# jgkellymit/GENIE-SMEM

Hardware: NVIDIA B200
Metric: SMEM reads/sec (BWA-SMEM; LUT/RMI under methods) (higher is better)
Workload: dtype u32

## Files before the change

genie_smem_b200/_capi.py:

```python
import ctypes as C
import os

_HERE = os.path.dirname(os.path.abspath(__file__))
LIB_PATH = os.path.join(_HERE, "libgenie_smem.so")

OK, E_INVALID, E_NOMEM, E_CUDA, E_CAPACITY, E_NODEVICE = 0, -1, -2, -3, -4, -5
METHOD_BWA, METHOD_LUT, METHOD_RMI = 0, 1, 2
READ_OK, READ_REF_RAISES, READ_TOO_SHORT = 0, 1, 2

u8p, u32p, u64p, i64p, f64p = (C.POINTER(t) for t in (C.c_uint8, C.c_uint32, C.c_uint64, C.c_int64, C.c_double))


class IndexInfo(C.Structure):
    _fields_ = [("n_bases", C.c_uint64), ("n_rows", C.c_uint64), ("n_buckets", C.c_uint64), ("bucket_bytes", C.c_uint64),
                ("text_words", C.c_uint64), ("count", C.c_uint32 * 4), ("C", C.c_uint32 * 5), ("primary_fwd", C.c_uint32),
                ("primary_rev", C.c_uint32), ("has_reverse", C.c_uint32), ("reserved", C.c_uint32)]


class DevIndex(C.Structure):
    _fields_ = [("n_rows", C.c_uint64), ("n_buckets", C.c_uint64), ("fwd_buckets", C.c_void_p), ("rev_buckets", C.c_void_p),
                ("sa", C.c_void_p), ("text2bit", C.c_void_p), ("C", C.c_uint32 * 5), ("primary_fwd", C.c_uint32),
                ("primary_rev", C.c_uint32), ("seed_K", C.c_uint32), ("seed_table", C.c_void_p)]


# ... 47 lines not shown
    "gsm_pack_reads": (C.c_int, [C.c_char_p, C.c_void_p, C.c_uint64, C.c_void_p, C.c_void_p]),
    "gsm_text_pack_device": (C.c_int, [C.c_void_p, C.c_uint64, C.c_uint32, C.c_void_p, C.c_void_p, C.c_void_p]),
    "gsm_index_build_device_workspace": (C.c_int, [C.c_uint64, C.c_uint32, C.POINTER(C.c_uint64)]),
    "gsm_index_build_device": (C.c_int, [C.c_void_p, C.c_uint64, C.c_uint32, C.c_void_p, C.c_void_p, C.c_void_p, C.c_void_p, C.c_uint64,
                                         C.POINTER(IndexInfo), C.c_void_p]),
    "gsm_fastq_scan": (C.c_int, [C.c_void_p, C.c_uint64, C.POINTER(C.c_uint64), C.c_void_p, C.c_void_p, C.c_uint64, C.c_uint32]),
    "gsm_fastq_gather": (C.c_int, [C.c_void_p, C.c_void_p, C.c_void_p, C.c_uint64, C.c_void_p, C.c_void_p, C.c_uint32]),
    "gsm_pack_reads_device": (C.c_int, [C.c_void_p, C.c_void_p, C.c_uint32, C.c_void_p, C.c_uint64, C.c_uint32, C.c_void_p, C.c_void_p, C.c_void_p,
                                        C.c_void_p]),
    "gsm_fastq_count_device": (C.c_int, [C.c_void_p, C.c_uint64, C.c_void_p, C.c_void_p]),
    "gsm_fastq_records_device": (C.c_int, [C.c_void_p, C.c_uint64, C.c_void_p, C.c_uint64, C.c_void_p, C.c_void_p, C.c_void_p, C.c_void_p]),
    "gsm_pack_reads_scattered_device": (C.c_int, [C.c_void_p, C.c_void_p, C.c_void_p, C.c_void_p, C.c_uint64, C.c_uint32, C.c_void_p, C.c_void_p,
                                                  C.c_void_p]),
    "gsm_pack_reads_device_check": (C.c_int, [C.c_void_p, C.c_void_p]),
    "gsm_reads_both_strands_device": (C.c_int, [C.POINTER(DevReads), C.c_void_p, C.c_void_p, C.c_void_p, C.c_void_p]),
    "gsm_smem_workspace_info": (C.c_int, [C.c_uint64, C.c_uint32, C.POINTER(WorkspaceInfo)]),
    "gsm_backsearch_batch": (C.c_int, [C.POINTER(DevIndex), C.POINTER(DevReads), C.c_void_p, C.c_void_p, C.c_void_p]),
    "gsm_backsearch_add_one_batch": (C.c_int, [C.POINTER(DevIndex), C.c_uint64, C.c_void_p, C.c_void_p, C.c_void_p, C.c_void_p]),
    "gsm_sa_lookup_batch": (C.c_int, [C.POINTER(DevIndex), C.c_uint64, C.c_void_p, C.c_void_p, C.c_void_p]),
    "gsm_sa_sample_build": (C.c_int, [C.POINTER(DevIndex), C.c_uint32, C.c_void_p, C.c_void_p]),
    "gsm_locate_sampled_batch": (C.c_int, [C.POINTER(DevIndex), C.c_void_p, C.c_uint32, C.c_uint64, C.c_void_p, C.c_void_p, C.c_void_p]),
    "gsm_lut_build": (C.c_int, [C.POINTER(DevIndex), C.c_uint32, C.c_void_p, C.c_void_p]),
    "gsm_seed_table_build": (C.c_int, [C.POINTER(DevIndex), C.c_uint32, C.c_void_p, C.c_void_p]),
    "gsm_smem_batch": (C.c_int, [C.c_int, C.POINTER(DevIndex), C.POINTER(DevReads), C.c_uint32, C.c_uint32, C.c_void_p,
                                 C.POINTER(DevRmi), C.POINTER(Workspace), C.c_void_p]),
    "gsm_smem_sweep": (C.c_int, [C.POINTER(DevIndex), C.POINTER(DevReads), C.POINTER(Workspace), C.c_void_p]),
    "gsm_smem_select": (C.c_int, [C.c_int, C.POINTER(DevIndex), C.POINTER(DevReads), C.c_uint32, C.c_uint32, C.c_void_p,
                                  C.POINTER(DevRmi), C.POINTER(Workspace), C.c_void_p]),
    "gsm_smem_collect": (C.c_int, [C.POINTER(DevReads), C.POINTER(Workspace), C.c_void_p, C.c_uint64, C.c_void_p]),
    "gsm_rmi_probe_build": (C.c_int, [C.POINTER(DevIndex), C.c_void_p, C.c_void_p]),
    "gsm_rmi_bounds_build": (C.c_int, [C.POINTER(DevIndex), C.c_uint32, C.c_void_p, C.c_void_p]),
    "gsm_option_lut_frame_machine": (C.c_int, [C.c_int]),
    "gsm_option_rmi_prefilter": (C.c_int, [C.c_int]),
    "gsm_rmi_hazard_scan": (C.c_int, [C.POINTER(DevIndex), C.POINTER(DevRmi), C.c_void_p, C.c_uint64, C.c_void_p, C.POINTER(C.c_uint64), C.c_void_p]),
    "gsm_rmi_hazard_hash": (C.c_int, [C.c_void_p, C.c_uint64, C.c_void_p, C.c_uint32]),
    "gsm_rmi_none_rows": (C.c_int, [C.POINTER(DevIndex), C.c_uint32, C.c_void_p, C.c_void_p, C.c_void_p]),
    "gsm_rmi_lookup_batch": (C.c_int, [C.POINTER(DevIndex), C.POINTER(DevRmi), C.c_uint64, C.c_void_p, C.c_void_p, C.c_void_p,
                                       C.c_void_p, C.c_void_p, C.c_void_p]),
    "gsm_comm_unique_id": (C.c_int, [C.c_void_p]),
    "gsm_comm_init": (C.c_int, [C.c_void_p, C.c_int, C.c_int, C.POINTER(C.c_void_p)]),
    "gsm_comm_free": (C.c_int, [C.c_void_p]),
    "gsm_comm_info": (C.c_int, [C.c_void_p, C.POINTER(C.c_int), C.POINTER(C.c_int), C.POINTER(C.c_int)]),
    "gsm_comm_allgather_u64": (C.c_int, [C.c_void_p, C.c_void_p, C.c_uint64, C.c_void_p, C.c_void_p]),
    "gsm_gather_records": (C.c_int, [C.c_void_p, C.c_void_p, C.c_uint64, C.c_void_p, C.c_void_p, C.c_int, C.c_void_p]),
    "gsm_peer_export": (C.c_int, [C.c_void_p, C.c_void_p, C.POINTER(C.c_uint64)]),
    "gsm_peer_open": (C.c_int, [C.c_void_p, C.c_uint64, C.POINTER(C.c_void_p)]),
    "gsm_peer_close": (C.c_int, [C.c_void_p, C.c_uint64]),
    "gsm_smem_collect_gathered": (C.c_int, [C.POINTER(DevReads), C.POINTER(Workspace), C.c_void_p, C.c_uint64, C.c_void_p, C.c_uint32,
                                            C.c_void_p, C.c_void_p]),
# ... 47 lines not shown
```

genie_smem_b200/csrc/kernels.cu:

```cuda
#include <cuda_runtime.h>

#include <algorithm>
#include <cstdint>
#include <cstdio>
#include <cstdlib>
#include <cstring>
#include <string>
#include <type_traits>

#include "../../include/genie_smem.h"
#include "host_common.hpp"
#include "select_logic.cuh"
#include "sweep_device.cuh"


namespace gsm {

#define GSM_CUDA(call)                                                                          \
    do {                                                                                        \
        cudaError_t e__ = (call);                                                               \
        if (e__ != cudaSuccess)                                                                 \
            return fail(GSM_E_CUDA, std::string(#call) + ": " + cudaGetErrorString(e__));       \
    } while (0)

// ... 847 lines not shown
    }
    table[code] = make_uint2(lo, cnt);
}

__global__ void k_seed_build(const uint4* fwd, const uint4* rev, IndexMeta meta, uint32_t K, uint64_t n_codes, uint4* table) {
    const uint64_t code = (uint64_t)blockIdx.x * blockDim.x + threadIdx.x;
    if (code >= n_codes) return;
    auto lf = [fwd](uint64_t idx) { return ldg_half(fwd, idx); };
    auto lr = [rev](uint64_t idx) { return ldg_half(rev, idx); };
    uint32_t lo = 0, cnt = meta.n_rows, rlo = 0, rcnt = meta.n_rows;
    for (uint32_t t = 0; t < K; ++t) {
        const uint32_t c = (uint32_t)(code >> (2 * t)) & 3u;
        const StepOut r = step_single(lf, lo, lo + cnt, c, meta.C[c], meta.prim_f);
        lo = r.lo_new; cnt = r.cnt_new;
    }
    for (uint32_t t = 0; t < K && rcnt && cnt; ++t) {
        const uint32_t c = (uint32_t)(code >> (2 * (K - 1 - t))) & 3u;
        const StepOut r = step_single(lr, rlo, rlo + rcnt, c, meta.C[c], meta.prim_r);
        rlo = r.lo_new; rcnt = r.cnt_new;
    }
    table[code] = make_uint4(lo, cnt, cnt ? rlo : 0u, 0u);
}

__global__ void k_bounds_build(const uint4* fwd, IndexMeta meta, uint32_t K, uint64_t n_codes, const uint4* seed_tab, uint32_t seed_K,
                               uint2* table) {
    const uint64_t code = (uint64_t)blockIdx.x * blockDim.x + threadIdx.x;
    if (code >= n_codes) return;
    auto load = [fwd](uint64_t idx) { return ldg_half(fwd, idx); };
    uint32_t lo = 0, cnt = meta.n_rows, t = 0;
    if (seed_tab) {
        const uint4 e = __ldg(seed_tab + (code & ((1ull << (2u * seed_K)) - 1ull)));
        lo = e.x; cnt = e.y; t = seed_K;
    }
    for (; t < K; ++t) {
        const uint32_t c = (uint32_t)(code >> (2 * t)) & 3u;
        const StepOut r = step_single(load, lo, lo + cnt, c, meta.C[c], meta.prim_f);
        lo = r.lo_new; cnt = r.cnt_new;
    }
    table[code] = make_uint2(lo, cnt);
}

__global__ void k_rmi_lookup(const uint32_t* sa, const uint32_t* text, uint64_t n_rows, uint64_t n_bases, RmiModel m, uint64_t n,
                             const uint64_t* codes, double* pred, int64_t* lo, int64_t* hi, uint8_t* status) {
    const uint64_t i = (uint64_t)blockIdx.x * blockDim.x + threadIdx.x;
    if (i >= n) return;
    auto sal = [sa](uint64_t r) { return __ldg(sa + r); };
// ... 327 lines not shown
        v.accessPolicyWindow.base_ptr = const_cast<void*>(ptr);
        v.accessPolicyWindow.num_bytes = (size_t)(bytes < (uint64_t)max_win ? bytes : (uint64_t)max_win);
        v.accessPolicyWindow.hitRatio = bytes <= carve ? 1.0f : (float)carve / (float)bytes;
        v.accessPolicyWindow.hitProp = cudaAccessPropertyPersisting;
        v.accessPolicyWindow.missProp = cudaAccessPropertyStreaming;
    }
    GSM_CUDA(cudaStreamSetAttribute((cudaStream_t)stream, cudaStreamAttributeAccessPolicyWindow, &v));
    if (!(ptr && bytes)) GSM_CUDA(cudaCtxResetPersistingL2Cache());
    return GSM_OK;
}

int gsm_seed_table_build(const gsm_dev_index* ix, uint32_t K, void* table, void* stream) {
    if (!ix || !table || !ix->fwd_buckets || !ix->rev_buckets) return fail(GSM_E_INVALID, "gsm_seed_table_build: needs both bucket arrays");
    if (K < 1 || K > 14) return fail(GSM_E_INVALID, "gsm_seed_table_build: K must be in 1..14");
    int st = device_ready();
    if (st) return st;
    const uint64_t n_codes = 1ull << (2 * K);
    k_seed_build<<<(unsigned)((n_codes + 127) / 128), 128, 0, (cudaStream_t)stream>>>((const uint4*)ix->fwd_buckets, (const uint4*)ix->rev_buckets,
                                                                                    make_meta(ix), K, n_codes, (uint4*)table);
    GSM_CUDA(cudaGetLastError());
    return GSM_OK;
}

static int fill_rmi(const gsm_dev_rmi* rmi, RmiModel* m, uint64_t n_rows) {
    memset(m, 0, sizeof(*m));
    if (!rmi || !rmi->level_sizes || !rmi->coef || !rmi->intercept) return fail(GSM_E_INVALID, "RMI parameters missing");
    if (rmi->n_levels < 1 || rmi->n_levels > 8 || rmi->K < 1 || rmi->K > 32) return fail(GSM_E_INVALID, "RMI: 1..8 levels, K in 1..32");
    m->K = rmi->K; m->n_levels = rmi->n_levels; m->coef = rmi->coef; m->intercept = rmi->intercept;
    m->stride = rmi->param_stride ? rmi->param_stride : 1u;
    uint32_t off = 0;
    for (uint32_t l = 0; l < rmi->n_levels; ++l) { m->level_size[l] = rmi->level_sizes[l]; m->level_off[l] = off; off += rmi->level_sizes[l]; }
    if (rmi->none_rows && rmi->n_none_rows) {
        if (rmi->n_none_rows != rmi->K) return fail(GSM_E_INVALID, "RMI: none_rows must hold exactly K rows (gsm_rmi_none_rows)");
        rmi_set_none_rows(*m, rmi->none_rows, rmi->n_none_rows, n_rows);
    }
    return GSM_OK;
}

int gsm_rmi_none_rows(const gsm_dev_index* ix, uint32_t K, uint32_t* rows_host, uint32_t* scratch, void* stream) {
    if (!ix || !ix->sa || !rows_host || !scratch || K < 1 || K > 32) return fail(GSM_E_INVALID, "gsm_rmi_none_rows: needs sa on the device, K in 1..32");
    int st = device_ready();
    if (st) return st;
    if (ix->n_rows <= K) return fail(GSM_E_INVALID, "gsm_rmi_none_rows: reference shorter than K");
    cudaStream_t s_ = (cudaStream_t)stream;
    GSM_CUDA(cudaMemsetAsync(scratch, 0, 33 * sizeof(uint32_t), s_));
    k_none_rows<<<(unsigned)((ix->n_rows + 255) / 256), 256, 0, s_>>>(ix->sa, ix->n_rows, K, scratch);
// ... 74 lines not shown
    GSM_CUDA(cudaGetLastError());
    return GSM_OK;
}

static int smem_check(const gsm_dev_index* ix, const gsm_dev_reads* rd, gsm_workspace* ws, int* sb, int* lb) {
    if (!ix || !rd || !ws) return fail(GSM_E_INVALID, "null");
    if (!ix->fwd_buckets || !ix->rev_buckets) return fail(GSM_E_INVALID, "the SMEM kernels need both BWT directions on the device");
    if (rd->max_len == 0 || rd->max_len > 65535) return fail(GSM_E_INVALID, "max_len must be in 1..65535");
    if (rd->n_reads >= (1ull << 32)) return fail(GSM_E_INVALID, "at most 2^32-1 reads per batch");
    if (ws->mem_cap >= (1ull << 32) || ws->rec_cap >= (1ull << 32)) return fail(GSM_E_INVALID, "pool capacities must be < 2^32 entries");
    int st = device_ready();
    if (st) return st;
    if ((st = sweep_grid(rd->max_len, sb))) return st;
    if ((st = select_grid(lb))) return st;
    const uint64_t need_sweep = sweep_scratch_bytes(*sb, rd->max_len);
    const uint64_t need_sel = (uint64_t)*lb * SELECT_THREADS * (uint64_t)select_stage_stride(rd->max_len) * 16ull;
    if (ws->quad_scratch_bytes < need_sweep || ws->quad_scratch_bytes < need_sel) return fail(GSM_E_CAPACITY, "quad_scratch too small (see gsm_smem_workspace_info)");
    const uint64_t n_tiles = (rd->n_reads + SCAN_TILE - 1) / SCAN_TILE;
    if (ws->scan_tmp_bytes < (n_tiles + 2) * 8) return fail(GSM_E_CAPACITY, "scan_tmp too small");
    return GSM_OK;
}

int gsm_smem_sweep(const gsm_dev_index* ix, const gsm_dev_reads* rd, gsm_workspace* ws, void* stream_) {
    int sb = 0, lb = 0;
    int st = smem_check(ix, rd, ws, &sb, &lb);
    if (st) return st;
    cudaStream_t stream = (cudaStream_t)stream_;
    GSM_CUDA(cudaMemsetAsync(ws->counters, 0, 8 * sizeof(uint64_t), stream));
    if (rd->n_reads == 0) return GSM_OK;
    SweepArgs sa;
    sa.fwd = (const uint4*)ix->fwd_buckets; sa.rev = (const uint4*)ix->rev_buckets; sa.meta = make_meta(ix);
    sa.reads = (const uint4*)rd->packed; sa.chunk_off = rd->chunk_off; sa.len = rd->len; sa.n_reads = (uint32_t)rd->n_reads;
    sa.read_u4 = sweep_read_u4(rd->max_len); sa.pack_u4 = sweep_pack_u4(rd->max_len); sa.max_len = rd->max_len;
    sa.seed_tab = (const uint4*)ix->seed_table; sa.seed_K = ix->seed_table ? ix->seed_K : 0u;
    if (sa.seed_tab && (sa.seed_K < 1 || sa.seed_K > 16)) return fail(GSM_E_INVALID, "seed table K must be in 1..16");
    sa.mem_pool = (uint4*)ws->mem_pool; sa.mem_cap = ws->mem_cap; sa.mem_off = ws->mem_off; sa.mem_cnt = ws->mem_cnt;
    sa.scratch = (uint4*)ws->quad_scratch; sa.counters = (unsigned long long*)ws->counters;
    static const int uniq_env = getenv("GSM_SWEEP_UNIQ") ? atoi(getenv("GSM_SWEEP_UNIQ")) : 1;
    sa.sa = ix->sa; sa.text = ix->text2bit; sa.n_bases = (uint32_t)(ix->n_rows - 1);
    const bool uniq = uniq_env != 0 && ix->sa && ix->text2bit;
    const int kind = sweep_kind(rd->max_len);
    if (kind == SWEEP_LANE) {
        static const int stats = getenv("GSM_SWEEP_STATS") ? atoi(getenv("GSM_SWEEP_STATS")) : 0;
        static const int paired = getenv("GSM_SWEEP_PAIRED") ? atoi(getenv("GSM_SWEEP_PAIRED")) : 0;
        if (uniq && paired) { k_sweep1<false, true, SWEEP1_MIN_BLOCKS, false, true><<<sb, SWEEP1_THREADS, sweep1_smem_bytes(rd->max_len, false), stream>>>(sa); GSM_CUDA(cudaGetLastError()); return GSM_OK; }
        if (uniq && stats) k_sweep1<false, true, SWEEP1_MIN_BLOCKS, true><<<sb, SWEEP1_THREADS, sweep1_smem_bytes(rd->max_len, false), stream>>>(sa);
        else if (uniq && sweep_blocks_env() == 6) k_sweep1<false, true, 6><<<sb, SWEEP1_THREADS, sweep1_smem_bytes(rd->max_len, false), stream>>>(sa);
        else if (uniq && sweep_blocks_env() == 8) k_sweep1<false, true, 8><<<sb, SWEEP1_THREADS, sweep1_smem_bytes(rd->max_len, false), stream>>>(sa);
        else if (uniq) k_sweep1<false, true><<<sb, SWEEP1_THREADS, sweep1_smem_bytes(rd->max_len, false), stream>>>(sa);
        else k_sweep1<false, false><<<sb, SWEEP1_THREADS, sweep1_smem_bytes(rd->max_len, false), stream>>>(sa);
    } else if (kind == SWEEP_LANE_LONG) {
        if (uniq) k_sweep1<true, true><<<sb, SWEEP1_THREADS, sweep1_smem_bytes(rd->max_len, true), stream>>>(sa);
        else k_sweep1<true, false><<<sb, SWEEP1_THREADS, sweep1_smem_bytes(rd->max_len, true), stream>>>(sa);
    } else {
        k_sweep<<<sb, SWEEP_THREADS, sweep_smem_bytes(rd->max_len), stream>>>(sa);
    }
    GSM_CUDA(cudaGetLastError());
    return GSM_OK;
// ... 203 lines not shown
```

genie_smem_b200/csrc/sweep_device.cuh:

```cuda
#pragma once
#include <cuda_runtime.h>

#include "sweep_logic.cuh"

namespace gsm {

constexpr int SWEEP_THREADS = 128;
constexpr int SWEEP_LPR = 2;
constexpr int SWEEP_GROUPS = SWEEP_THREADS / SWEEP_LPR;
constexpr int SWEEP_CAP = 12;
constexpr int SWEEP_MIN_BLOCKS = 8;

constexpr uint32_t MEMS_ORDERED = 0x80000000u;
constexpr uint32_t MEMS_PICKED = 0x40000000u;
constexpr uint32_t MEMS_COUNT = 0x3FFFFFFFu;

struct SweepArgs {
    const uint4* fwd;
    const uint4* rev;
    IndexMeta meta;
    const uint4* reads;
    const uint32_t* chunk_off;
    const uint32_t* len;
    uint32_t n_reads;
    uint32_t read_u4;
    uint32_t pack_u4;
    uint32_t max_len;
    const uint4* seed_tab;
    uint32_t seed_K;
    uint4* mem_pool;
    unsigned long long mem_cap;
    uint32_t* mem_off;
    uint32_t* mem_cnt;
    uint4* scratch;
    unsigned long long* counters;
    const uint32_t* sa;
    const uint32_t* text;
    uint32_t n_bases;
};

extern __shared__ uint4 g_sweep_smem[];

__device__ __forceinline__ Half ldg_half(const uint4* halves_base, size_t half_index) {
    Half h;
    asm volatile("ld.global.nc.v8.u32 {%0,%1,%2,%3,%4,%5,%6,%7}, [%8];"
                 : "=r"(h.c0), "=r"(h.c1), "=r"(h.l0), "=r"(h.l1), "=r"(h.l2), "=r"(h.h0), "=r"(h.h1), "=r"(h.h2)
                 : "l"(halves_base + half_index * 2));
    return h;
}

__device__ __forceinline__ StepOut pair_step(const uint4* __restrict__ bk, uint32_t P0, uint32_t P1, uint32_t ch, uint32_t Cc,
// ... 99 lines not shown
        if (g == 0) { a.mem_off[rid] = (uint32_t)off; a.mem_cnt[rid] = n; }
    }
};

__host__ __device__ inline uint32_t sweep_read_u4(uint32_t max_len) { return (max_len + 15u) / 16u; }

__global__ void __launch_bounds__(SWEEP_THREADS, SWEEP_MIN_BLOCKS) k_sweep(const SweepArgs a) {
    const uint32_t lane = threadIdx.x & 31u;
    const uint32_t g = lane & 1u;
    const uint32_t pair_in_block = threadIdx.x >> 1;
    const uint32_t pair_u4 = SWEEP_CAP + a.read_u4 + a.pack_u4;
    const uint32_t p0 = pair_in_block * pair_u4;
    const size_t gp = (size_t)blockIdx.x * SWEEP_GROUPS + pair_in_block;
    DevSweepCtx ctx{a, p0, (p0 + SWEEP_CAP) * 16u, (p0 + SWEEP_CAP + a.read_u4) * 4u, a.scratch + gp * 2 * a.max_len,
                    a.scratch + gp * 2 * a.max_len + a.max_len, g, 3u << (lane & ~1u), lane & ~1u};
    Sweeper<DevSweepCtx> sw;
    for (;;) {
        const bool need = sw.next(ctx, a.meta);
        if (!__any_sync(0xFFFFFFFFu, need)) break;
        const bool is_seed = need && sw.pending_seed();
        const bool is_step = need && !is_seed;
        uint4 se = make_uint4(0u, 0u, 0u, 0u);
        if (is_seed) se = ldg_seed(a.seed_tab + sw.P0);
        const bool rev = sw.on_reverse();
        const StepOut r = pair_step(rev ? a.rev : a.fwd, sw.P0, sw.P0 + sw.cnt, sw.ch, a.meta.C[sw.ch & 3u],
                                    rev ? a.meta.prim_r : a.meta.prim_f, g, is_step);
        if (is_step) sw.consume(ctx, a.meta, r);
        else if (is_seed) sw.consume_seed(ctx, a.meta, SeedEntry{se.x, se.y, se.z, se.w});
    }
}

constexpr int SWEEP1_THREADS = 128;
constexpr int SWEEP1_CAP = 8;
constexpr int SWEEP1_MIN_BLOCKS = 7;

struct LanePartial {
    uint32_t eq0, lt0;
    bool have;
};

template <bool PAIRED>
__device__ __forceinline__ bool lane_step(const uint4* __restrict__ fwd, const uint4* __restrict__ rev, bool use_rev, uint32_t P0, uint32_t P1,
                                          uint32_t ch, uint32_t Cc, uint32_t primary, bool active, LanePartial& part, StepOut& out) {
    constexpr uint32_t FULLM = 0xFFFFFFFFu;
    uint32_t b0, r0, b1, r1;
    split192(P0, b0, r0);
// ... 223 lines not shown

template <bool LONG, bool UNIQ, int MB = SWEEP1_MIN_BLOCKS, bool STATS = false, bool PAIRED = false>
__global__ void __launch_bounds__(SWEEP1_THREADS, MB) k_sweep1(const SweepArgs a) {
    using Ctx = DevSweepCtx1<LONG, UNIQ>;
    const uint32_t lane_u4 = sweep1_lane_u4(a.max_len, LONG);
    const uint32_t p0 = threadIdx.x * lane_u4;
    const size_t gl = (size_t)blockIdx.x * SWEEP1_THREADS + threadIdx.x;
    Ctx ctx{a, p0, (p0 + SWEEP1_CAP) * 4u, a.scratch + gl * 2 * a.max_len, a.scratch + gl * 2 * a.max_len + a.max_len, nullptr, 0u, Ctx::NO_FIN};
    Sweeper<Ctx> sw;
    LanePartial part{0u, 0u, false};
    uint32_t n_it = 0, n_step = 0, n_seed = 0, n_text = 0;
    for (;;) {
        ctx.flush_finished();
        const bool need = sw.next(ctx, a.meta);
        if (__any_sync(0xFFFFFFFFu, ctx.fin_n != Ctx::NO_FIN)) ctx.flush_finished();
        if (!__any_sync(0xFFFFFFFFu, need)) break;
        const bool is_seed = need && sw.pending_seed();
        const bool is_word = UNIQ && need && sw.pending_word();
        const bool is_cmp = UNIQ && need && sw.pending_cmp();
        const bool is_step = need && !is_seed && !is_word && !is_cmp;
        if (STATS) { n_it++; n_step += is_step; n_seed += is_seed; n_text += is_word || is_cmp; }
        uint4 se = make_uint4(0u, 0u, 0u, 0u);
        if (is_seed) se = ldg_seed(a.seed_tab + sw.P0);
        uint32_t wv = 0u, matched = 0u;
        if (UNIQ && is_word) wv = __ldg(a.sa + sw.aux);
        if (UNIQ && is_cmp) {
            matched = ctx.match_forward(sw.cmp_text(), sw.cmp_read());
            const uint32_t mx = sw.cmp_max(a.n_bases);
            matched = matched < mx ? matched : mx;
        }
        const bool rev = sw.on_reverse();
        StepOut r;
        const bool stepped = lane_step<PAIRED>(a.fwd, a.rev, rev, sw.P0, sw.P0 + sw.cnt, sw.ch, a.meta.C[sw.ch & 3u],
                                               rev ? a.meta.prim_r : a.meta.prim_f, is_step, part, r);
        if (stepped) sw.consume(ctx, a.meta, r);
        else if (is_seed) sw.consume_seed(ctx, a.meta, SeedEntry{se.x, se.y, se.z, se.w});
        else if (UNIQ && is_word) sw.consume_word(ctx, a.meta, wv);
        else if (UNIQ && is_cmp) sw.consume_cmp(ctx, a.meta, matched);
    }
    if (STATS) {
        atomicAdd(&a.counters[4], (unsigned long long)n_it);
        atomicAdd(&a.counters[5], (unsigned long long)n_step);
        atomicAdd(&a.counters[6], (unsigned long long)n_seed);
        atomicAdd(&a.counters[7], (unsigned long long)n_text);
    }
}
// ... 9 lines not shown
```

genie_smem_b200/csrc/sweep_logic.cuh:

```cuda
#pragma once
#include "fm_core.cuh"

namespace gsm {

struct IndexMeta {
    uint32_t C[4];
    uint32_t cnt[4];
    uint32_t prim_f, prim_r;
    uint32_t n_rows;
};

struct MemEntry {
    uint32_t se, lo, cnt, sweep;
};

struct SeedEntry {
    uint32_t fwd_lo, cnt, rev_lo, pad;
};

enum SweepMode : int { M_FETCH = 0, M_FWD = 1, M_WALK = 2, M_SEEDF = 3, M_SEEDB = 4, M_DONE = 5,
                       M_SAF = 6,
                       M_SAW = 7,
                       M_CMPF = 8,
                       M_CMPB = 9,
                       M_ISA = 10 };

constexpr uint32_t SWEEP_CMP_CHUNK = 64;

GSM_HD uint32_t bwa_pick_key(uint32_t start, uint32_t end, uint32_t k, uint32_t p) {
    if (end <= p) return 0u;
    return (start <= p ? 0x80000000u | ((end - start) << 6) : 0u) | (63u - k);
}
GSM_HD uint32_t bwa_pick_of(uint32_t key) { return 63u - (key & 63u); }

template <typename Ctx>
struct Sweeper {
    int mode = M_FETCH;
    uint32_t rid = 0, L = 0;
    uint32_t x = 0, F = 0, lb = 0;
    uint32_t n_mems = 0, sweep_id = 0;
    uint32_t P0 = 0, cnt = 0, ch = 0;
// ... 108 lines not shown
        ncand--;
        c.cand_get(ncand, cur_j, P0, cnt);
        F = cur_j;
        last_start = 0xFFFFFFFFu;
        if (x == 0) {
            emit_match(c, 0, cur_j, P0, cnt);
            end_sweep(c);
            return;
        }
        if (cnt == 1u && x != lb && c.uniq() && c.uniq_back()) {
            pos = x;
            if (have_tpos) uniq_walk_next(c, m);
            else { aux = P0; mode = M_SAW; }
            return;
        }
        walk_from(c, m, x);
    }

    GSM_HD bool try_walk(Ctx& c, uint32_t start) {
        if (start == lb || start == 0) return false;
        pos = start - 1;
        ch = c.base(pos);
        mode = M_WALK;
        return true;
    }

    GSM_HD void walk_from(Ctx& c, const IndexMeta& m, uint32_t start) {
        if (!try_walk(c, start)) walk_end(c, m, start);
    }

    GSM_HD void walk_end(Ctx& c, const IndexMeta& m, uint32_t start) {
        for (;;) {
            if (start < last_start) emit_match(c, start, cur_j, P0, cnt);
            if (start == lb || (ncand == 0 && short_hi <= x)) { end_sweep(c); return; }
            if (ncand != 0) {
                ncand--;
                c.cand_get(ncand, cur_j, P0, cnt);
                start = x;
            } else {
                cur_j = short_hi--;
                const uint32_t K = c.seed_k();
                if (cur_j >= K && cur_j - K >= lb) { P0 = c.kmer(cur_j - K); mode = M_SEEDB; return; }
                start = plain_begin(c, m);
            }
            if (try_walk(c, start)) return;
        }
// ... 3 lines not shown
        const uint32_t b = c.base(cur_j - 1);
        P0 = m.C[b]; cnt = m.cnt[b];
        return cur_j - 1;
    }

    GSM_HD bool next(Ctx& c, const IndexMeta& m) {
        while (mode == M_FETCH) {
            if (x >= L) {
                if (!c.fetch(rid, L)) { mode = M_DONE; return false; }
                n_mems = 0; sweep_id = 0; x = 0; lb = 0;
                if (L == 0) { c.finish(rid, 0); continue; }
            }
            start_sweep(c, m);
        }
        return mode != M_DONE;
    }

    GSM_HD void consume_seed(Ctx& c, const IndexMeta& m, const SeedEntry& e) {
        if (mode == M_SEEDF) {
            if (e.cnt == 0) { fwd_plain(c, m); return; }
            k = e.fwd_lo; P0 = e.rev_lo; cnt = e.cnt;
            pos = x + c.seed_k();
            short_hi = pos - 1;
            fwd_continue(c, m);
            return;
        }
        if (e.cnt == 0) { walk_from(c, m, plain_begin(c, m)); return; }
        P0 = e.fwd_lo; cnt = e.cnt;
        walk_from(c, m, cur_j - c.seed_k());
    }

    GSM_HD void consume(Ctx& c, const IndexMeta& m, const StepOut& r) {
        const bool fwd = mode == M_FWD;
        if (fwd && r.cnt_new != cnt) c.cand_put(ncand++, pos, k, cnt);
        if (r.cnt_new != 0) {
            k += r.lt_add; P0 = r.lo_new; cnt = r.cnt_new;
            const bool more = fwd ? (pos + 1u != L) : (pos != lb && pos != 0u);
            if (more && !(fwd && cnt == 1u && c.uniq())) { pos += fwd ? 1u : 0xFFFFFFFFu; ch = c.base(pos); return; }
            if (fwd) {
                pos++;
                fwd_continue(c, m);
                return;
            }
            walk_end(c, m, pos);
            return;
        }
        if (fwd) start_bwd(c, m);
        else walk_end(c, m, pos + 1u);
    }
};

}
```

genie_smem_b200/engine.py:

```python
import ctypes as C

import numpy as np
import torch

from . import _capi as capi
from .ingest import Contigs

RECORD_DTYPE = np.dtype([("read_id", "<u4"), ("qstart", "<u2"), ("qend", "<u2"), ("sa_lo", "<u4"), ("sa_hi", "<u4")])
HIT_DTYPE = np.dtype([("record", "<u4"), ("contig", "<u4"), ("offset", "<u4"), ("flags", "<u4")])
CHAIN_DTYPE = np.dtype([("slot", "<u4"), ("contig", "<u4"), ("rbeg", "<u4"), ("rend", "<u4"), ("q", "<u4"), ("weight", "<u4"),
                        ("n_seeds", "<u4"), ("reserved", "<u4")])
_BASES = np.frombuffer(b"ACGT", dtype=np.uint8)


class BaseError(KeyError, ValueError):
    """A read or reference holds a character outside ACGT (the reference raises KeyError there,
    SMEM/ExactMatch.py:139; SURVEY 8b asks for ValueError up front -- this is both)."""


def _ptr(t):
    return C.c_void_p(t.data_ptr()) if t is not None else C.c_void_p(0)


def _stream():
# ... 221 lines not shown
            if verify and (zlib.crc32(memoryview(a).cast("B")) & 0xFFFFFFFF) != d["crc32"]:
                raise ValueError(f"{path}: section {d['name']} is corrupt (CRC-32 mismatch)")
            arrs[d["name"]] = a
        info = capi.IndexInfo()
        for k in PackedIndex.FIELDS:
            setattr(info, k, head["info"][k])
        for c in range(4):
            info.count[c] = head["info"]["count"][c]
        for c in range(5):
            info.C[c] = head["info"]["C"][c]
        dev = torch.device(device)

        def up(name):
            a = arrs.get(name)
            return None if a is None else torch.from_numpy(np.array(a)).to(dev)
        index = DeviceIndex.__new__(DeviceIndex)
        index.device, index.info, index.build_stats = dev, info, None
        index.fwd, index.rev, index.sa, index.text = up("fwd"), up("rev"), up("sa"), up("text")
        if "ssa" in arrs:
            index.ssa, index.sa_sample = up("ssa"), head["sa_sample"]
        if "seed_table" in arrs:
            index.seed_table, index.seed_K = up("seed_table"), head["seed_K"]
        index._bind()
        if "contigs" in head:
            index.set_contigs(Contigs(head["contigs"], np.array(arrs["contig_start"])))
        lut = up("lut")
        rmi = None
        if head["rmi"] is not None:
            p = np.array(arrs["rmi_params"])
            rmi = RmiParams(head["rmi"]["K"], head["rmi"]["level_sizes"], p[:, 0], p[:, 1], dev)
            rmi.max_err = head["rmi"]["max_err"]
            if head["rmi"]["none_rows"] is not None:
                rows = np.asarray(head["rmi"]["none_rows"], np.uint32)
                rmi.none_rows = rows
                rmi.c.none_rows = rows.ctypes.data_as(capi.u32p)
                rmi.c.n_none_rows = len(rows)
            if "rmi_probe" in arrs:
                rmi.probe = up("rmi_probe")
                rmi.c.probe = rmi.probe.data_ptr()
        return index, lut, head["lut_K"], rmi


class DeviceIndex:

    contigs = None
    _contig_start = None
# ... 71 lines not shown
            ws = torch.empty(int(need.value), dtype=torch.uint8, device=dev)
            self.info = capi.IndexInfo()
            e1.record()
            capi.check(capi.lib.gsm_index_build_device(_ptr(self.text), n_bases, flags, _ptr(self.sa), _ptr(self.fwd), _ptr(self.rev),
                                                       _ptr(ws), int(need.value), C.byref(self.info), _stream()))
            e2.record()
            torch.cuda.synchronize(dev)
            del ws
            torch.cuda.empty_cache()
        self.build_stats = {"pack_ms": e0.elapsed_time(e1), "build_ms": e1.elapsed_time(e2), "workspace_bytes": int(need.value),
                            "doubling_rounds": int(self.info.reserved)}
        self.info.reserved = 0
        self._bind()
        return self

    def build_seed_table(self, K=None):
        if K is None:
            K = 1
            while K < 14 and self.n_rows / 4.0 ** (K + 1) >= 2.0:
                K += 1
        if self.rev is None:
            raise ValueError("the seed table needs the reverse-text buckets")
        K = int(K)
        self.seed_table, self.seed_K = None, 0
        self._bind()
        t = torch.empty((1 << (2 * K)) * 4, dtype=torch.int32, device=self.device)
        with torch.cuda.device(self.device):
            capi.check(capi.lib.gsm_seed_table_build(C.byref(self.c), K, _ptr(t), _stream()))
        self.seed_table, self.seed_K = t, K
        self._bind()
        return self

    def build_sampled_sa(self, sample=32, drop_full=False):
        if self.sa is None:
            raise ValueError("the sampled suffix array is derived from the full one")
        n = (self.n_rows + sample - 1) // sample
        self.ssa = torch.empty(n, dtype=torch.int32, device=self.device)
        self.sa_sample = int(sample)
        with torch.cuda.device(self.device):
            capi.check(capi.lib.gsm_sa_sample_build(C.byref(self.c), self.sa_sample, _ptr(self.ssa), _stream()))
        if drop_full:
            torch.cuda.synchronize(self.device)
            self.sa = None
            self._bind()
        return self

    def locate(self, rows):
        rows = np.ascontiguousarray(rows, np.uint32)
        if rows.size == 0:
            return np.zeros(0, np.uint32)
        if self.sa is not None:
            return sa_lookup(self, rows)
        if getattr(self, "ssa", None) is None:
            raise ValueError("no suffix array on the device: call build_sampled_sa() before dropping it")
        with torch.cuda.device(self.device):
            r = torch.from_numpy(rows.view(np.int32)).to(self.device)
            out = torch.empty_like(r)
            capi.check(capi.lib.gsm_locate_sampled_batch(C.byref(self.c), _ptr(self.ssa), self.sa_sample, rows.size, _ptr(r), _ptr(out), _stream()))
        return out.cpu().numpy().view(np.uint32)

    def set_contigs(self, contigs):
        if contigs is None:
            self.contigs, self._contig_start, self._contigs_c = None, None, None
            return self
        if contigs.n_bases != self.n_bases:
            raise ValueError(f"contigs cover {contigs.n_bases} bases, the index {self.n_bases}")
        self._contig_start = torch.from_numpy(contigs.start.view(np.int32).copy()).to(self.device)
        self._contigs_c = capi.DevContigs(len(contigs), self._contig_start.data_ptr())
        self.contigs = contigs
        return self

    def drop_seed_table(self):
        self.seed_table, self.seed_K = None, 0
        self._bind()
        return self

    def suffix_array_host(self):
        return self.sa.cpu().numpy().view(np.uint32)

    def count_dic(self):
        i = self.info
        return {"": int(i.n_rows), "$": 0, "A": int(i.C[0]), "C": int(i.C[1]), "G": int(i.C[2]), "T": int(i.C[3])}

    def bytes(self):
        return sum(t.numel() * t.element_size() for t in (self.fwd, self.rev, self.sa, self.text, getattr(self, "seed_table", None)) if t is not None)


class ReadBatch:

    def __init__(self, packed_u8, chunk_off, lens, max_len, read_id_base=0):
        self.packed_host, self.chunk_off_host, self.len_host = packed_u8, chunk_off, lens
        self.n = int(lens.shape[0])
        self.max_len = int(max_len)
        self.read_id_base = int(read_id_base)
        self.packed = self.chunk_off = self.len = None

    @classmethod
    def from_strings(cls, reads, read_id_base=0, pin=False):
        lens = np.asarray([len(r) for r in reads], np.uint32)
        joined = "".join(reads).encode()
        return cls._pack(joined, lens, read_id_base, pin)

    @classmethod
    def from_codes(cls, codes_u8, read_len, read_id_base=0, pin=False):
        n = codes_u8.shape[0]
        lens = np.full(n, read_len, np.uint32)
        joined = _BASES[np.ascontiguousarray(codes_u8).reshape(-1)].tobytes()
        return cls._pack(joined, lens, read_id_base, pin)
# ... 345 lines not shown
            m = max(self.max_reads, 1)
            self.ds_packed = torch.empty(2 * m * ((self.max_len + 63) // 64) * 16 + 16, dtype=torch.uint8, device=dev)
            self.ds_chunk_off = torch.empty(2 * m + 1, dtype=torch.int32, device=dev)
            self.ds_len = torch.empty(2 * m, dtype=torch.int32, device=dev)

    def _both_strands(self, reads):
        if reads.n > self.max_reads or reads.max_len > self.max_len:
            raise ValueError("batch exceeds the engine's workspace")
        _check_doubled_ids(reads.read_id_base, reads.n)
        capi.check(capi.lib.gsm_reads_both_strands_device(C.byref(reads.cstruct()), _ptr(self.ds_packed), _ptr(self.ds_chunk_off),
                                                          _ptr(self.ds_len), _stream()))
        self.kernel_launches += 1
        return _ChunkView(self.ds_packed, self.ds_chunk_off, self.ds_len, 2 * reads.n, reads.max_len, 2 * reads.read_id_base,
                          2 * getattr(reads, "lo", 0))

    def _check_batch(self, reads):
        if reads.n > self.slots or reads.max_len > self.max_len:
            raise ValueError("batch exceeds the engine's workspace")
        self._reads_c = reads.cstruct()
        return self._reads_c

    def sweep(self, reads: ReadBatch):
        r = self._check_batch(reads)
        capi.check(capi.lib.gsm_smem_sweep(C.byref(self.index.c), C.byref(r), C.byref(self.ws), _stream()))
        self.kernel_launches += 1 if reads.n else 0

    def select(self, method, reads: ReadBatch, min_len=1, K=0, lut=None, rmi: RmiParams = None, gatherer=None):
        if gatherer is not None and self.strands == 2:
            raise ValueError("strands=2 does not support a gatherer")
        r = self._check_batch(reads)
        capi.check(capi.lib.gsm_smem_select(method, C.byref(self.index.c), C.byref(r), int(min_len), int(K), _ptr(lut),
                                            C.byref(rmi.c) if rmi is not None else None, C.byref(self.ws), _stream()))
        pre = 2 if (reads.n and method == capi.METHOD_RMI and rmi is not None and rmi.hazard_slots is not None and rmi.bounds is not None
                    and capi.lib.gsm_option_rmi_prefilter(-1) != 0) else 0
        if gatherer is not None:
            gatherer.collect(self, r)
            self.kernel_launches += ((8 if self._picks_path(method) else 7) + pre) if reads.n else 1
            return
        capi.check(capi.lib.gsm_smem_collect(C.byref(r), C.byref(self.ws), _ptr(self.records), self.rec_cap, _stream()))
        self.kernel_launches += ((7 if self._picks_path(method) else 6) + pre) if reads.n else 0

    @staticmethod
    def _picks_path(method):
        return method == capi.METHOD_BWA or (method == capi.METHOD_LUT and capi.lib.gsm_option_lut_frame_machine(-1) == 0)

    def collect_local(self, reads: ReadBatch):
        r = self._check_batch(reads)
# ... 636 lines not shown
```

include/genie_smem.h:

```cpp
#ifndef GENIE_SMEM_H
#define GENIE_SMEM_H

#include <stdint.h>

#ifdef __cplusplus
extern "C" {
#endif

#define GSM_OK 0
#define GSM_E_INVALID (-1)
#define GSM_E_NOMEM (-2)
#define GSM_E_CUDA (-3)
#define GSM_E_CAPACITY (-4)
#define GSM_E_NODEVICE (-5)

#define GSM_METHOD_BWA 0
#define GSM_METHOD_LUT 1
#define GSM_METHOD_RMI 2

#define GSM_READ_OK 0u
#define GSM_READ_REF_RAISES 1u
#define GSM_READ_TOO_SHORT 2u

#define GSM_BUCKET_BYTES 64
// ... 130 lines not shown
    uint32_t grid_blocks;
    uint32_t block_threads;
} gsm_workspace_info;

int gsm_smem_workspace_info(uint64_t n_reads, uint32_t max_len, gsm_workspace_info* out);

int gsm_backsearch_batch(const gsm_dev_index* idx, const gsm_dev_reads* reads, uint32_t* lo,
                         uint32_t* cnt, void* stream);

int gsm_backsearch_add_one_batch(const gsm_dev_index* idx, uint64_t n, const uint8_t* base,
                                 uint32_t* lo, uint32_t* cnt, void* stream);

int gsm_sa_lookup_batch(const gsm_dev_index* idx, uint64_t n, const uint32_t* rows, uint32_t* pos,
                        void* stream);

int gsm_sa_sample_build(const gsm_dev_index* idx, uint32_t sample, uint32_t* ssa, void* stream);
int gsm_locate_sampled_batch(const gsm_dev_index* idx, const uint32_t* ssa, uint32_t sample, uint64_t n,
                             const uint32_t* rows, uint32_t* pos, void* stream);

int gsm_lut_build(const gsm_dev_index* idx, uint32_t K, uint32_t* table, void* stream);

int gsm_seed_table_build(const gsm_dev_index* idx, uint32_t K, void* table, void* stream);

int gsm_smem_batch(int method, const gsm_dev_index* idx, const gsm_dev_reads* reads, uint32_t min_len,
                   uint32_t K, const uint32_t* lut, const gsm_dev_rmi* rmi, gsm_workspace* ws,
                   void* stream);

int gsm_option_lut_frame_machine(int on);

int gsm_smem_sweep(const gsm_dev_index* idx, const gsm_dev_reads* reads, gsm_workspace* ws, void* stream);
int gsm_smem_select(int method, const gsm_dev_index* idx, const gsm_dev_reads* reads, uint32_t min_len,
                    uint32_t K, const uint32_t* lut, const gsm_dev_rmi* rmi, gsm_workspace* ws,
                    void* stream);

int gsm_smem_collect(const gsm_dev_reads* reads, gsm_workspace* ws, gsm_record* out, uint64_t out_cap,
                     void* stream);

typedef struct gsm_comm gsm_comm;
int gsm_comm_unique_id(void* id128);
int gsm_comm_init(const void* id128, int rank, int world, gsm_comm** out);
int gsm_comm_free(gsm_comm* comm);
int gsm_comm_info(const gsm_comm* comm, int* rank, int* world, int* nccl_version);
int gsm_comm_allgather_u64(gsm_comm* comm, const uint64_t* send_dev, uint64_t n, uint64_t* recv_dev, void* stream);
int gsm_gather_records(gsm_comm* comm, const gsm_record* send, uint64_t n_send, const uint64_t* counts, gsm_record* recv,
                       int dst, void* stream);
int gsm_peer_export(const void* dev_ptr, void* handle64, uint64_t* offset);
int gsm_peer_open(const void* handle64, uint64_t offset, void** dev_ptr);
int gsm_peer_close(void* dev_ptr, uint64_t offset);
int gsm_smem_collect_gathered(const gsm_dev_reads* reads, gsm_workspace* ws, gsm_record* out, uint64_t out_cap,
                              const uint64_t* counts_dev, uint32_t rank, const uint64_t* base_dev, void* stream);
int gsm_gather_advance(uint64_t* base_dev, const uint64_t* counts_dev, uint32_t world, void* stream);

int gsm_rmi_probe_build(const gsm_dev_index* idx, void* probe, void* stream);
// ... 79 lines not shown
```

Baseline: 217.6 million.

## Precompute seed extension dead-masks to skip doomed FM-index steps in sweep

Adds a per-seed-code bitmask table recording which one- and two-base left extensions and one-base right extensions yield an empty interval. The sweep state machine reads the mask with the seed entry and ends walks or forward extension early instead of issuing an occ-lookup step that is known to fail. This removes dependent bucket loads per SMEM at the cost of an extra 4-byte gather per seed hit, a one-time build kernel, and more memory for the mask table.

```diff
diff --git a/genie_smem_b200/_capi.py b/genie_smem_b200/_capi.py
--- a/genie_smem_b200/_capi.py
+++ b/genie_smem_b200/_capi.py
@@ -93,9 +93,11 @@
     "gsm_locate_sampled_batch": (C.c_int, [C.POINTER(DevIndex), C.c_void_p, C.c_uint32, C.c_uint64, C.c_void_p, C.c_void_p, C.c_void_p]),
     "gsm_lut_build": (C.c_int, [C.POINTER(DevIndex), C.c_uint32, C.c_void_p, C.c_void_p]),
     "gsm_seed_table_build": (C.c_int, [C.POINTER(DevIndex), C.c_uint32, C.c_void_p, C.c_void_p]),
+    "gsm_seed_ext_build": (C.c_int, [C.POINTER(DevIndex), C.c_void_p, C.c_void_p]),
     "gsm_smem_batch": (C.c_int, [C.c_int, C.POINTER(DevIndex), C.POINTER(DevReads), C.c_uint32, C.c_uint32, C.c_void_p,
                                  C.POINTER(DevRmi), C.POINTER(Workspace), C.c_void_p]),
     "gsm_smem_sweep": (C.c_int, [C.POINTER(DevIndex), C.POINTER(DevReads), C.POINTER(Workspace), C.c_void_p]),
+    "gsm_smem_sweep_ext": (C.c_int, [C.POINTER(DevIndex), C.c_void_p, C.POINTER(DevReads), C.POINTER(Workspace), C.c_void_p]),
     "gsm_smem_select": (C.c_int, [C.c_int, C.POINTER(DevIndex), C.POINTER(DevReads), C.c_uint32, C.c_uint32, C.c_void_p,
                                   C.POINTER(DevRmi), C.POINTER(Workspace), C.c_void_p]),
     "gsm_smem_collect": (C.c_int, [C.POINTER(DevReads), C.POINTER(Workspace), C.c_void_p, C.c_uint64, C.c_void_p]),
diff --git a/genie_smem_b200/csrc/kernels.cu b/genie_smem_b200/csrc/kernels.cu
--- a/genie_smem_b200/csrc/kernels.cu
+++ b/genie_smem_b200/csrc/kernels.cu
@@ -893,6 +893,26 @@
     table[code] = make_uint4(lo, cnt, cnt ? rlo : 0u, 0u);
 }
 
+__global__ void k_seed_ext_build(const uint4* fwd, const uint4* rev, IndexMeta meta, uint64_t n_codes, const uint4* table, uint32_t* ext) {
+    const uint64_t code = (uint64_t)blockIdx.x * blockDim.x + threadIdx.x;
+    if (code >= n_codes) return;
+    auto lf = [fwd](uint64_t idx) { return ldg_half(fwd, idx); };
+    auto lr = [rev](uint64_t idx) { return ldg_half(rev, idx); };
+    const uint4 e = __ldg(table + code);
+    uint32_t dead = 0;
+    if (e.y) {
+        for (uint32_t b1 = 0; b1 < 4u; ++b1) {
+            const StepOut s = step_single(lf, e.x, e.x + e.y, b1, meta.C[b1], meta.prim_f);
+            if (s.cnt_new == 0) { dead |= (1u << b1) | (0xFu << (SEED_DEAD_LEFT2 + 4u * b1)); continue; }
+            for (uint32_t b2 = 0; b2 < 4u; ++b2)
+                if (!step_single(lf, s.lo_new, s.lo_new + s.cnt_new, b2, meta.C[b2], meta.prim_f).cnt_new) dead |= 1u << (SEED_DEAD_LEFT2 + 4u * b1 + b2);
+        }
+        for (uint32_t r = 0; r < 4u; ++r)
+            if (!step_single(lr, e.z, e.z + e.y, r, meta.C[r], meta.prim_r).cnt_new) dead |= 1u << (SEED_DEAD_RIGHT + r);
+    }
+    ext[code] = dead;
+}
+
 __global__ void k_bounds_build(const uint4* fwd, IndexMeta meta, uint32_t K, uint64_t n_codes, const uint4* seed_tab, uint32_t seed_K,
                                uint2* table) {
     const uint64_t code = (uint64_t)blockIdx.x * blockDim.x + threadIdx.x;
@@ -1266,6 +1286,18 @@
     return GSM_OK;
 }
 
+int gsm_seed_ext_build(const gsm_dev_index* ix, uint32_t* ext, void* stream) {
+    if (!ix || !ext || !ix->fwd_buckets || !ix->rev_buckets || !ix->seed_table) return fail(GSM_E_INVALID, "gsm_seed_ext_build: needs both bucket arrays and the seed table");
+    if (ix->seed_K < 1 || ix->seed_K > 14) return fail(GSM_E_INVALID, "gsm_seed_ext_build: seed_K must be in 1..14");
+    int st = device_ready();
+    if (st) return st;
+    const uint64_t n_codes = 1ull << (2 * ix->seed_K);
+    k_seed_ext_build<<<(unsigned)((n_codes + 127) / 128), 128, 0, (cudaStream_t)stream>>>((const uint4*)ix->fwd_buckets, (const uint4*)ix->rev_buckets,
+                                                                                        make_meta(ix), n_codes, (const uint4*)ix->seed_table, ext);
+    GSM_CUDA(cudaGetLastError());
+    return GSM_OK;
+}
+
 static int fill_rmi(const gsm_dev_rmi* rmi, RmiModel* m, uint64_t n_rows) {
     memset(m, 0, sizeof(*m));
     if (!rmi || !rmi->level_sizes || !rmi->coef || !rmi->intercept) return fail(GSM_E_INVALID, "RMI parameters missing");
@@ -1386,9 +1418,14 @@
 }
 
 int gsm_smem_sweep(const gsm_dev_index* ix, const gsm_dev_reads* rd, gsm_workspace* ws, void* stream_) {
+    return gsm_smem_sweep_ext(ix, nullptr, rd, ws, stream_);
+}
+
+int gsm_smem_sweep_ext(const gsm_dev_index* ix, const uint32_t* seed_ext, const gsm_dev_reads* rd, gsm_workspace* ws, void* stream_) {
     int sb = 0, lb = 0;
     int st = smem_check(ix, rd, ws, &sb, &lb);
     if (st) return st;
+    if (seed_ext && !ix->seed_table) return fail(GSM_E_INVALID, "gsm_smem_sweep_ext: extension masks without a seed table");
     cudaStream_t stream = (cudaStream_t)stream_;
     GSM_CUDA(cudaMemsetAsync(ws->counters, 0, 8 * sizeof(uint64_t), stream));
     if (rd->n_reads == 0) return GSM_OK;
@@ -1398,6 +1435,7 @@
     sa.read_u4 = sweep_read_u4(rd->max_len); sa.pack_u4 = sweep_pack_u4(rd->max_len); sa.max_len = rd->max_len;
     sa.seed_tab = (const uint4*)ix->seed_table; sa.seed_K = ix->seed_table ? ix->seed_K : 0u;
     if (sa.seed_tab && (sa.seed_K < 1 || sa.seed_K > 16)) return fail(GSM_E_INVALID, "seed table K must be in 1..16");
+    sa.seed_ext = seed_ext;
     sa.mem_pool = (uint4*)ws->mem_pool; sa.mem_cap = ws->mem_cap; sa.mem_off = ws->mem_off; sa.mem_cnt = ws->mem_cnt;
     sa.scratch = (uint4*)ws->quad_scratch; sa.counters = (unsigned long long*)ws->counters;
     static const int uniq_env = getenv("GSM_SWEEP_UNIQ") ? atoi(getenv("GSM_SWEEP_UNIQ")) : 1;
diff --git a/genie_smem_b200/csrc/sweep_device.cuh b/genie_smem_b200/csrc/sweep_device.cuh
--- a/genie_smem_b200/csrc/sweep_device.cuh
+++ b/genie_smem_b200/csrc/sweep_device.cuh
@@ -27,6 +27,7 @@
     uint32_t pack_u4;
     uint32_t max_len;
     const uint4* seed_tab;
+    const uint32_t* seed_ext;
     uint32_t seed_K;
     uint4* mem_pool;
     unsigned long long mem_cap;
@@ -172,6 +173,7 @@
         const bool is_step = need && !is_seed;
         uint4 se = make_uint4(0u, 0u, 0u, 0u);
         if (is_seed) se = ldg_seed(a.seed_tab + sw.P0);
+        if (is_seed && a.seed_ext) se.w = __ldg(a.seed_ext + sw.P0);
         const bool rev = sw.on_reverse();
         const StepOut r = pair_step(rev ? a.rev : a.fwd, sw.P0, sw.P0 + sw.cnt, sw.ch, a.meta.C[sw.ch & 3u],
                                     rev ? a.meta.prim_r : a.meta.prim_f, g, is_step);
@@ -441,6 +443,7 @@
         if (STATS) { n_it++; n_step += is_step; n_seed += is_seed; n_text += is_word || is_cmp; }
         uint4 se = make_uint4(0u, 0u, 0u, 0u);
         if (is_seed) se = ldg_seed(a.seed_tab + sw.P0);
+        if (is_seed && a.seed_ext) se.w = __ldg(a.seed_ext + sw.P0);
         uint32_t wv = 0u, matched = 0u;
         if (UNIQ && is_word) wv = __ldg(a.sa + sw.aux);
         if (UNIQ && is_cmp) {
diff --git a/genie_smem_b200/csrc/sweep_logic.cuh b/genie_smem_b200/csrc/sweep_logic.cuh
--- a/genie_smem_b200/csrc/sweep_logic.cuh
+++ b/genie_smem_b200/csrc/sweep_logic.cuh
@@ -15,8 +15,9 @@
 };
 
 struct SeedEntry {
-    uint32_t fwd_lo, cnt, rev_lo, pad;
-};
+    uint32_t fwd_lo, cnt, rev_lo, dead;
+};
+constexpr uint32_t SEED_DEAD_LEFT2 = 4, SEED_DEAD_RIGHT = 20;
 
 enum SweepMode : int { M_FETCH = 0, M_FWD = 1, M_WALK = 2, M_SEEDF = 3, M_SEEDB = 4, M_DONE = 5,
                        M_SAF = 6,
@@ -171,6 +172,7 @@
         pos = start - 1;
         ch = c.base(pos);
         mode = M_WALK;
+        aux = 0;
         return true;
     }
 
@@ -220,12 +222,15 @@
             k = e.fwd_lo; P0 = e.rev_lo; cnt = e.cnt;
             pos = x + c.seed_k();
             short_hi = pos - 1;
+            if (pos < L && ((e.dead >> (SEED_DEAD_RIGHT + c.base(pos))) & 1u)) { c.cand_put(ncand++, pos, k, cnt); start_bwd(c, m); return; }
             fwd_continue(c, m);
             return;
         }
         if (e.cnt == 0) { walk_from(c, m, plain_begin(c, m)); return; }
         P0 = e.fwd_lo; cnt = e.cnt;
-        walk_from(c, m, cur_j - c.seed_k());
+        const uint32_t start = cur_j - c.seed_k();
+        if (!try_walk(c, start) || ((e.dead >> ch) & 1u)) { walk_end(c, m, start); return; }
+        aux = (e.dead >> (SEED_DEAD_LEFT2 + 4u * ch)) & 0xFu;
     }
 
     GSM_HD void consume(Ctx& c, const IndexMeta& m, const StepOut& r) {
@@ -234,14 +239,19 @@
         if (r.cnt_new != 0) {
             k += r.lt_add; P0 = r.lo_new; cnt = r.cnt_new;
             const bool more = fwd ? (pos + 1u != L) : (pos != lb && pos != 0u);
-            if (more && !(fwd && cnt == 1u && c.uniq())) { pos += fwd ? 1u : 0xFFFFFFFFu; ch = c.base(pos); return; }
-            if (fwd) {
+            if (more && !(fwd && cnt == 1u && c.uniq())) {
+                const uint32_t dead = fwd ? 0u : aux;
+                aux = 0;
+                pos += fwd ? 1u : 0xFFFFFFFFu; ch = c.base(pos);
+                if (!((dead >> ch) & 1u)) return;
+            } else if (fwd) {
                 pos++;
                 fwd_continue(c, m);
                 return;
+            } else {
+                walk_end(c, m, pos);
+                return;
             }
-            walk_end(c, m, pos);
-            return;
         }
         if (fwd) start_bwd(c, m);
         else walk_end(c, m, pos + 1u);
diff --git a/genie_smem_b200/engine.py b/genie_smem_b200/engine.py
--- a/genie_smem_b200/engine.py
+++ b/genie_smem_b200/engine.py
@@ -267,6 +267,8 @@
         if "seed_table" in arrs:
             index.seed_table, index.seed_K = up("seed_table"), head["seed_K"]
         index._bind()
+        if "seed_table" in arrs:
+            index.build_seed_ext()
         if "contigs" in head:
             index.set_contigs(Contigs(head["contigs"], np.array(arrs["contig_start"])))
         lut = up("lut")
@@ -384,14 +386,36 @@
         if self.rev is None:
             raise ValueError("the seed table needs the reverse-text buckets")
         K = int(K)
-        self.seed_table, self.seed_K = None, 0
+        self.seed_table, self.seed_K, self.seed_ext = None, 0, None
         self._bind()
         t = torch.empty((1 << (2 * K)) * 4, dtype=torch.int32, device=self.device)
+        e0, e1 = torch.cuda.Event(enable_timing=True), torch.cuda.Event(enable_timing=True)
         with torch.cuda.device(self.device):
+            e0.record()
             capi.check(capi.lib.gsm_seed_table_build(C.byref(self.c), K, _ptr(t), _stream()))
+            e1.record()
+            e1.synchronize()
+        self.build_stats = dict(getattr(self, "build_stats", None) or {}, seed_table_ms=e0.elapsed_time(e1))
         self.seed_table, self.seed_K = t, K
         self._bind()
+        return self.build_seed_ext()
+
+    def build_seed_ext(self):
+        self.seed_ext = None
+        t = torch.empty(1 << (2 * self.seed_K), dtype=torch.int32, device=self.device)
+        e0, e1 = torch.cuda.Event(enable_timing=True), torch.cuda.Event(enable_timing=True)
+        with torch.cuda.device(self.device):
+            e0.record()
+            capi.check(capi.lib.gsm_seed_ext_build(C.byref(self.c), _ptr(t), _stream()))
+            e1.record()
+            e1.synchronize()
+        self.build_stats = dict(getattr(self, "build_stats", None) or {}, seed_ext_ms=e0.elapsed_time(e1))
+        self.seed_ext = t
         return self
+
+    def seed_ext_ptr(self):
+        ext, tab = getattr(self, "seed_ext", None), getattr(self, "seed_table", None)
+        return ext.data_ptr() if ext is not None and tab is not None and ext.numel() * 4 == tab.numel() else None
 
     def build_sampled_sa(self, sample=32, drop_full=False):
         if self.sa is None:
@@ -433,7 +457,7 @@
         return self
 
     def drop_seed_table(self):
-        self.seed_table, self.seed_K = None, 0
+        self.seed_table, self.seed_K, self.seed_ext = None, 0, None
         self._bind()
         return self
 
@@ -445,7 +469,7 @@
         return {"": int(i.n_rows), "$": 0, "A": int(i.C[0]), "C": int(i.C[1]), "G": int(i.C[2]), "T": int(i.C[3])}
 
     def bytes(self):
-        return sum(t.numel() * t.element_size() for t in (self.fwd, self.rev, self.sa, self.text, getattr(self, "seed_table", None)) if t is not None)
+        return sum(t.numel() * t.element_size() for t in (self.fwd, self.rev, self.sa, self.text, getattr(self, "seed_table", None), getattr(self, "seed_ext", None)) if t is not None)
 
 
 class ReadBatch:
@@ -837,7 +861,7 @@
 
     def sweep(self, reads: ReadBatch):
         r = self._check_batch(reads)
-        capi.check(capi.lib.gsm_smem_sweep(C.byref(self.index.c), C.byref(r), C.byref(self.ws), _stream()))
+        capi.check(capi.lib.gsm_smem_sweep_ext(C.byref(self.index.c), self.index.seed_ext_ptr(), C.byref(r), C.byref(self.ws), _stream()))
         self.kernel_launches += 1 if reads.n else 0
 
     def select(self, method, reads: ReadBatch, min_len=1, K=0, lut=None, rmi: RmiParams = None, gatherer=None):
diff --git a/include/genie_smem.h b/include/genie_smem.h
--- a/include/genie_smem.h
+++ b/include/genie_smem.h
@@ -176,6 +176,8 @@
 
 int gsm_seed_table_build(const gsm_dev_index* idx, uint32_t K, void* table, void* stream);
 
+int gsm_seed_ext_build(const gsm_dev_index* idx, uint32_t* ext, void* stream);
+
 int gsm_smem_batch(int method, const gsm_dev_index* idx, const gsm_dev_reads* reads, uint32_t min_len,
                    uint32_t K, const uint32_t* lut, const gsm_dev_rmi* rmi, gsm_workspace* ws,
                    void* stream);
@@ -183,6 +185,7 @@
 int gsm_option_lut_frame_machine(int on);
 
 int gsm_smem_sweep(const gsm_dev_index* idx, const gsm_dev_reads* reads, gsm_workspace* ws, void* stream);
+int gsm_smem_sweep_ext(const gsm_dev_index* idx, const uint32_t* seed_ext, const gsm_dev_reads* reads, gsm_workspace* ws, void* stream);
 int gsm_smem_select(int method, const gsm_dev_index* idx, const gsm_dev_reads* reads, uint32_t min_len,
                     uint32_t K, const uint32_t* lut, const gsm_dev_rmi* rmi, gsm_workspace* ws,
                     void* stream);
```

Result: slower. 188.8 million, median of 6 (-13.2%).
